# ChristianFeldmann/libHM

Hardware: AMD Instinct MI355X
Metric: decoded Mpixels/s (luma), 2160p Main10 reconstruction + loop filters (higher is better)
Workload: dtype int16 samples / int32 accumulate; 1 GPU; 3840x2160 Main10 lowdelay_P pictures, pre-parsed CTU metadata: prep+MC+dequant/IT/recon+deblock+SAO, batch of 16 independent pictures per step, inputs resident in HBM; sub_benchmark=full, streams=2, parallelism=frame-parallel, 1 process per GPU, no data-path collective

## Files before the change

libhm_amd/csrc/filter_core.h:

```cpp
#pragma once
#include "hmgpu_dev.h"

namespace hmgpu {

static __constant__ uint8_t c_tc_table[54] = {0, 0, 0, 0, 0, 0, 0, 0, 0, 0, 0, 0, 0, 0, 0, 0, 0, 0, 1, 1, 1, 1, 1, 1, 1, 1, 1,
                                       2, 2, 2, 2, 3, 3, 3, 3, 4, 4, 4, 5, 5, 6, 6, 7, 8, 9, 10, 11, 13, 14, 16, 18, 20, 22, 24};
static __constant__ uint8_t c_beta_table[52] = {0, 0, 0, 0, 0, 0, 0, 0, 0, 0, 0, 0, 0, 0, 0, 0, 6, 7, 8, 9, 10, 11, 12, 13, 14, 15,
                                         16, 17, 18, 20, 22, 24, 26, 28, 30, 32, 34, 36, 38, 40, 42, 44, 46, 48, 50, 52, 54,
                                         56, 58, 60, 62, 64};
static __constant__ uint8_t c_chroma_scale_420_dbk[58] = {
    0, 1, 2, 3, 4, 5, 6, 7, 8, 9, 10, 11, 12, 13, 14, 15, 16, 17, 18, 19, 20, 21, 22, 23, 24, 25, 26, 27, 28, 29,
    29, 30, 31, 32, 33, 33, 34, 34, 35, 35, 36, 36, 37, 37, 38, 39, 40, 41, 42, 43, 44, 45, 46, 47, 48, 49, 50, 51};

__device__ inline bool mvd4(const int16_t* a, const int16_t* b) { return abs(a[0] - b[0]) >= 4 || abs(a[1] - b[1]) >= 4; }
typedef short mv2 __attribute__((ext_vector_type(2)));
__device__ inline bool mvd4(uint32_t a, uint32_t b) {
  const mv2 d = __builtin_elementwise_sub_sat(__builtin_bit_cast(mv2, a), __builtin_bit_cast(mv2, b));
  const mv2 m = __builtin_elementwise_max(d, __builtin_elementwise_sub_sat((mv2){0, 0}, d));
  return (__builtin_bit_cast(uint32_t, m) & 0xfffcfffcu) != 0u;
}

__device__ inline int boundary_strength(const BlkInfo& p, const BlkInfo& q, bool transform_edge) {
  if ((p.flags | q.flags) & BF_INTRA) return 2;
  if (transform_edge && ((p.flags | q.flags) & BF_CBFY)) return 1;
  const int p0 = p.ref[0], p1 = p.ref[1], q0 = q.ref[0], q1 = q.ref[1];
  if ((p0 == q0 && p1 == q1) || (p0 == q1 && p1 == q0)) {
    const uint32_t pm0 = __builtin_bit_cast(uint32_t, *reinterpret_cast<const mv2*>(p.mv[0])), pm1 = __builtin_bit_cast(uint32_t, *reinterpret_cast<const mv2*>(p.mv[1]));
    const uint32_t qm0 = __builtin_bit_cast(uint32_t, *reinterpret_cast<const mv2*>(q.mv[0])), qm1 = __builtin_bit_cast(uint32_t, *reinterpret_cast<const mv2*>(q.mv[1]));
    const bool straight = mvd4(qm0, pm0) || mvd4(qm1, pm1), crossed = mvd4(qm1, pm0) || mvd4(qm0, pm1);
    if (p0 != p1) return (p0 == q0 ? straight : crossed) ? 1 : 0;
    return (straight && crossed) ? 1 : 0;
  }
  return 1;
}

typedef short s16x2 __attribute__((ext_vector_type(2)));
typedef unsigned short u16x2 __attribute__((ext_vector_type(2)));
__device__ inline s16x2 as_s16x2(uint32_t v) { return __builtin_bit_cast(s16x2, v); }
__device__ inline u16x2 as_u16x2(uint32_t v) { return __builtin_bit_cast(u16x2, v); }
__device__ inline uint32_t as_u32(s16x2 v) { return __builtin_bit_cast(uint32_t, v); }
__device__ inline uint32_t as_u32(u16x2 v) { return __builtin_bit_cast(uint32_t, v); }
__device__ inline s16x2 splat(int v) { return (s16x2){(short)v, (short)v}; }
__device__ inline u16x2 usplat(int v) { return (u16x2){(unsigned short)v, (unsigned short)v}; }
__device__ inline s16x2 pk_clip(s16x2 lo, s16x2 hi, s16x2 v) { return __builtin_elementwise_min(__builtin_elementwise_max(v, lo), hi); }

__device__ inline void filter_luma_pair_strong(uint32_t (&s)[8], int tc) {
  const u16x2 m0 = as_u16x2(s[0]), m1 = as_u16x2(s[1]), m2 = as_u16x2(s[2]), m3 = as_u16x2(s[3]);
  const u16x2 m4 = as_u16x2(s[4]), m5 = as_u16x2(s[5]), m6 = as_u16x2(s[6]), m7 = as_u16x2(s[7]);
  const s16x2 t2 = splat(2 * tc);
  const u16x2 s23 = m2 + m3, s34 = m3 + m4, s45 = m4 + m5;
  const u16x2 n3 = (m1 + s23 + s23 + m4 + m4 + m5 + usplat(4)) >> 3;
  const u16x2 n4 = (m2 + s34 + s34 + m5 + m5 + m6 + usplat(4)) >> 3;
  const u16x2 n2 = (m1 + s23 + m4 + usplat(2)) >> 2;
  const u16x2 n5 = (s34 + m5 + m6 + usplat(2)) >> 2;
  const u16x2 n1 = (m0 + m0 + m1 + m1 + m1 + s23 + m4 + usplat(4)) >> 3;
  const u16x2 n6 = (s34 + m5 + m6 + m6 + m6 + m7 + m7 + usplat(4)) >> 3;
  (void)s45;
  auto lim = [&](u16x2 m, u16x2 n) { const s16x2 c = as_s16x2(as_u32(m)); return as_u32(pk_clip(c - t2, c + t2, as_s16x2(as_u32(n)))); };
  s[1] = lim(m1, n1); s[2] = lim(m2, n2); s[3] = lim(m3, n3);
  s[4] = lim(m4, n4); s[5] = lim(m5, n5); s[6] = lim(m6, n6);
}
__device__ inline void filter_luma_pair_weak(uint32_t (&s)[8], int tc, int thr_cut, bool filt_p, bool filt_q, int maxv, bool wide) {
  const s16x2 m1 = as_s16x2(s[1]), m2 = as_s16x2(s[2]), m3 = as_s16x2(s[3]), m4 = as_s16x2(s[4]), m5 = as_s16x2(s[5]), m6 = as_s16x2(s[6]);
  const s16x2 zero = splat(0), mx = splat(maxv), tcv = splat(tc), tc2 = splat(tc >> 1);
  s16x2 delta;
  if (wide) {
    const int lo = (9 * ((int)m4.x - (int)m3.x) - 3 * ((int)m5.x - (int)m2.x) + 8) >> 4;
    const int hi = (9 * ((int)m4.y - (int)m3.y) - 3 * ((int)m5.y - (int)m2.y) + 8) >> 4;
    delta = (s16x2){(short)lo, (short)hi};
  } else {
    delta = ((m4 - m3) * splat(9) - (m5 - m2) * splat(3) + splat(8)) >> 4;
  }
  const uint32_t on = as_u32((__builtin_elementwise_max(delta, -delta) - splat(thr_cut)) >> 15);
  delta = pk_clip(-tcv, tcv, delta);
  const uint32_t n3 = as_u32(pk_clip(zero, mx, m3 + delta)), n4 = as_u32(pk_clip(zero, mx, m4 - delta));
  s[3] = (n3 & on) | (s[3] & ~on);
  s[4] = (n4 & on) | (s[4] & ~on);
  if (filt_p) {
    const s16x2 d1 = pk_clip(-tc2, tc2, ((((m1 + m3 + splat(1)) >> 1) - m2 + delta) >> 1));
    s[2] = (as_u32(pk_clip(zero, mx, m2 + d1)) & on) | (s[2] & ~on);
  }
  if (filt_q) {
    const s16x2 d2 = pk_clip(-tc2, tc2, ((((m6 + m4 + splat(1)) >> 1) - m5 - delta) >> 1));
    s[5] = (as_u32(pk_clip(zero, mx, m5 + d2)) & on) | (s[5] & ~on);
  }
}

__device__ inline void filter_luma_unit(uint32_t (&a)[8], uint32_t (&b)[8], int bs, int qp, int tc_offset_div2, int beta_offset_div2, int bd,
                                        bool p_nofilt = false, bool q_nofilt = false) {
  const int scale = 1 << (bd - 8);
  const int tc = c_tc_table[clip3(0, 53, qp + 2 * (bs - 1) + (tc_offset_div2 << 1))] * scale;
  const int beta = c_beta_table[clip3(0, 51, qp + (beta_offset_div2 << 1))] * scale;
  const int side = (beta + (beta >> 1)) >> 3;
  int l0[8], l3[8];
#pragma unroll
  for (int k = 0; k < 8; k++) { l0[k] = (int)(a[k] & 0xffffu); l3[k] = (int)(b[k] >> 16); }
  const int dp0 = abs(l0[1] - 2 * l0[2] + l0[3]), dq0 = abs(l0[4] - 2 * l0[5] + l0[6]);
  const int dp3 = abs(l3[1] - 2 * l3[2] + l3[3]), dq3 = abs(l3[4] - 2 * l3[5] + l3[6]);
  const int d0 = dp0 + dq0, d3 = dp3 + dq3, d = d0 + d3;
  if (d >= beta) return;
  const bool fp = (dp0 + dp3) < side, fq = (dq0 + dq3) < side;
  const bool s0 = (abs(l0[0] - l0[3]) + abs(l0[7] - l0[4]) < (beta >> 3)) && (2 * d0 < (beta >> 2)) &&
                  (abs(l0[3] - l0[4]) < ((tc * 5 + 1) >> 1));
  const bool s3 = (abs(l3[0] - l3[3]) + abs(l3[7] - l3[4]) < (beta >> 3)) && (2 * d3 < (beta >> 2)) &&
                  (abs(l3[3] - l3[4]) < ((tc * 5 + 1) >> 1));
  const int maxv = (1 << bd) - 1;
  uint32_t ka[8], kb[8];
#pragma unroll
  for (int k = 0; k < 8; k++) { ka[k] = a[k]; kb[k] = b[k]; }
  if (s0 && s3) {
    filter_luma_pair_strong(a, tc);
    filter_luma_pair_strong(b, tc);
  } else {
    filter_luma_pair_weak(a, tc, tc * 10, fp, fq, maxv, bd > 10);
    filter_luma_pair_weak(b, tc, tc * 10, fp, fq, maxv, bd > 10);
  }
#pragma unroll
  for (int k = 0; k < 4; k++) {
    if (p_nofilt) { a[k] = ka[k]; b[k] = kb[k]; }
    if (q_nofilt) { a[4 + k] = ka[4 + k]; b[4 + k] = kb[4 + k]; }
  }
}

__device__ inline void rows_to_pairs(const uint32_t (&r0)[4], const uint32_t (&r1)[4], uint32_t (&a)[8]) {
#pragma unroll
  for (int j = 0; j < 4; j++) {
    a[2 * j] = __builtin_amdgcn_perm(r1[j], r0[j], 0x05040100u);
    a[2 * j + 1] = __builtin_amdgcn_perm(r1[j], r0[j], 0x07060302u);
  }
}
__device__ inline void pairs_to_rows(const uint32_t (&a)[8], uint32_t (&r0)[4], uint32_t (&r1)[4]) {
#pragma unroll
  for (int j = 0; j < 4; j++) {
    r0[j] = __builtin_amdgcn_perm(a[2 * j + 1], a[2 * j], 0x05040100u);
    r1[j] = __builtin_amdgcn_perm(a[2 * j + 1], a[2 * j], 0x07060302u);
  }
}

__device__ inline int chroma_tc(int qp_avg, int pps_off, int tc_offset_div2, int bd, int fmt = 1) {
  int qp = qp_avg + pps_off;
  if (qp >= 58) qp = fmt == 1 ? qp - 6 : min(qp, 51);
  else if (qp >= 0) qp = fmt == 1 ? c_chroma_scale_420_dbk[qp] : min(qp, 51);
  return c_tc_table[clip3(0, 53, qp + 2 + (tc_offset_div2 << 1))] * (1 << (bd - 8));
}



template <int DX>
__device__ inline void shifted(const u32x4 e, uint32_t l, uint32_t r, uint32_t (&n)[4]) {
  if constexpr (DX == 0) { n[0] = e.x; n[1] = e.y; n[2] = e.z; n[3] = e.w; }
  else if constexpr (DX < 0) {
    n[0] = (e.x << 16) | l; n[1] = __builtin_amdgcn_alignbit(e.y, e.x, 16);
    n[2] = __builtin_amdgcn_alignbit(e.z, e.y, 16); n[3] = __builtin_amdgcn_alignbit(e.w, e.z, 16);
  } else {
    n[0] = __builtin_amdgcn_alignbit(e.y, e.x, 16); n[1] = __builtin_amdgcn_alignbit(e.z, e.y, 16);
    n[2] = __builtin_amdgcn_alignbit(e.w, e.z, 16); n[3] = (e.w >> 16) | (r << 16);
  }
}

__device__ inline s16x2 lut_offsets(uint32_t idx_pk, uint32_t tab_lo, uint32_t tab_hi) {
  const uint32_t looked = __builtin_amdgcn_perm(tab_hi, tab_lo, idx_pk << 8);
  return as_s16x2(__builtin_amdgcn_perm(0u, looked, 0x09030801u));
}

__device__ inline void sao_exempt_mask(const PicDev& P, int comp, int x, int row, uint32_t (&m)[4]) {
  const int sx = comp ? P.csx : 0, sy = comp ? P.csy : 0;
  const BlkInfo* g = P.blk + (size_t)((row << sy) >> 2) * P.grid_w + ((x << sx) >> 2);
#pragma unroll
  for (int j = 0; j < 4; j++) {
    const int blk = sx ? j : (j >> 1);
    m[j] = (ldg(&g[blk].flags) & BF_NOFILT) ? 0xffffffffu : 0u;
  }
}

__device__ inline u32x4 ldc8(const int16_t* row_c, int x, int comp) {
  const int16_t* p = row_c - (comp - 1) + kCStep * x;
  const u32x4 a = ldg4(p), b = ldg4(p + 8);
  const uint32_t sel = comp == 2 ? 0x07060302u : 0x05040100u;
  return u32x4{__builtin_amdgcn_perm(a.y, a.x, sel), __builtin_amdgcn_perm(a.w, a.z, sel), __builtin_amdgcn_perm(b.y, b.x, sel), __builtin_amdgcn_perm(b.w, b.z, sel)};
}
__device__ inline void stc8(int16_t* row_c, int x, const u32x4 v) {
  int16_t* p = row_c + kCStep * x;
  const uint32_t w[4] = {v.x, v.y, v.z, v.w};
#pragma unroll
  for (int j = 0; j < 4; j++) { stg(p + kCStep * 2 * j, (int16_t)(w[j] & 0xffffu)); stg(p + kCStep * (2 * j + 1), (int16_t)(w[j] >> 16)); }
}

template <int DX, int DY>
__device__ inline void sao_eo_core(int x, int row, const u32x4 cur, const uint32_t (&na)[4], const uint32_t (&nb)[4], uint32_t off_lo, uint32_t off_hi,
                                   unsigned av, int x0, int y0, int x1, int y1, int maxv, uint32_t (&out)[4]) {
  const int ya = row + DY, yb = row - DY;
  const int va = ya < y0 ? 0 : (ya > y1 ? 2 : 1), vb = yb < y0 ? 0 : (yb > y1 ? 2 : 1);
  const unsigned ra = av >> (3 * va), rb = av >> (3 * vb);
  const bool mid_ok = ((ra & rb) >> 1) & 1;
  const int last = min(7, x1 - x);
  const int ha0 = (x + DX) < x0 ? 0 : 1, hb0 = (x - DX) < x0 ? 0 : 1;
  const int hal = (x + last + DX) > x1 ? 2 : 1, hbl = (x + last - DX) > x1 ? 2 : 1;
  const bool ok0 = ((ra >> ha0) & (rb >> hb0)) & 1;
  const bool okl = ((ra >> hal) & (rb >> hbl)) & 1;
  const uint32_t c[4] = {cur.x, cur.y, cur.z, cur.w};
  const uint32_t midm = mid_ok ? 0xffffffffu : 0u;
  const uint32_t lastm = (midm & 0x0000ffffu) | (okl ? 0xffff0000u : 0u);
  uint32_t m[4] = {midm, midm, midm, midm};
  if constexpr (DX != 0) {
    m[0] = (midm & 0xffff0000u) | (ok0 ? 0x0000ffffu : 0u);
    m[1] = last == 3 ? lastm : midm;
    m[3] = last == 3 ? midm : lastm;
  }
  uint32_t one_u = 0x00010001u, mone_u = 0xffffffffu;
  asm("" : "+v"(one_u));
  asm("" : "+v"(mone_u));
  const s16x2 one = as_s16x2(one_u), mone = as_s16x2(mone_u);
#pragma unroll
  for (int j = 0; j < 4; j++) {
    const s16x2 cc = as_s16x2(c[j]);
    const s16x2 sa = __builtin_elementwise_max(__builtin_elementwise_min(cc - as_s16x2(na[j]), one), mone);
    const s16x2 sb = __builtin_elementwise_max(__builtin_elementwise_min(cc - as_s16x2(nb[j]), one), mone);
    const uint32_t et = as_u32(sa + sb + splat(2));
    const s16x2 off = lut_offsets(et, off_lo, off_hi);
    const s16x2 res = __builtin_elementwise_min(__builtin_elementwise_max(cc + off, splat(0)), splat(maxv));
    out[j] = (as_u32(res) & m[j]) | (c[j] & ~m[j]);
  }
}

}
```

libhm_amd/csrc/k_filter.hip:

```cpp
#include "hmgpu_dev.h"
#include "filter_core.h"
#include <type_traits>

namespace hmgpu {

namespace {
constexpr int kTW = 64, kTH = 64;
constexpr int kYC = kTW + 16, kYH = kTH + 8;
constexpr int kCC = kTW / 2 + 16, kCH = kTH / 2 + 4;
constexpr int kYW = kYC + 8, kCW = kCC + 8;

constexpr int kUnits = 9 * 18;
struct FilterLds {
  __attribute__((aligned(16))) int16_t y[kYH][kYW];
  __attribute__((aligned(16))) int16_t c[2][kCH][kCW];
  uint32_t unit[2][3][64];
  int32_t units[2][4];
};

struct SaoPrm { uint32_t w0, off_lo, off_hi; };
__device__ inline SaoPrm sao_fetch(const PicDev& P, int comp, int x, int row) {
  const int log2ctb = P.log2ctu - (comp ? 1 : 0);
  const int w = P.width >> (comp ? 1 : 0), h = P.height >> (comp ? 1 : 0);
  SaoPrm r = {0xffu, 0u, 0u};
  if (x < w && row < h) {
    const uint32_t* pw = reinterpret_cast<const uint32_t*>(P.saoprm + ((size_t)(row >> log2ctb) * P.ctus_w + (x >> log2ctb)) * 3 + comp);
    r.w0 = ldg(pw); r.off_lo = ldg(pw + 1); r.off_hi = ldg(pw + 2);
  }
  return r;
}

template <int W, bool NF>
__device__ inline u32x4 sao_group(const PicDev& P, int comp, const int16_t (*t)[W], int ox, int oy, int x, int row, const SaoPrm& prm) {
  const int cs = comp ? 1 : 0;
  const int w = P.width >> cs, h = P.height >> cs;
  const int log2ctb = P.log2ctu - cs;
  const int cx = x >> log2ctb, cy = row >> log2ctb;
  const uint32_t w0 = prm.w0;
  const int type = (int)(int8_t)(w0 & 0xff);
  const int16_t* line = &t[row - oy][x - ox];
  const u32x4 cur = *reinterpret_cast<const u32x4*>(line);
  if (type < 0) return cur;
  const uint32_t off_lo = prm.off_lo, off_hi = prm.off_hi;
  const int bd = P.bd[comp], maxv = (1 << bd) - 1;
  uint32_t out[4];
  if (type == HMGPU_SAO_BO) {
    const int shift = bd - 5, band0 = (w0 >> 8) & 0xff;
    const uint32_t c[4] = {cur.x, cur.y, cur.z, cur.w};
#pragma unroll
    for (int j = 0; j < 4; j++) {
      const uint32_t lo = c[j] & 0xffffu, hi = c[j] >> 16;
      const uint32_t k0 = min(((lo >> shift) - band0) & 31u, 4u), k1 = min(((hi >> shift) - band0) & 31u, 4u);
      const s16x2 off = lut_offsets(k0 | (k1 << 16), off_lo, 0u);
      out[j] = as_u32(__builtin_elementwise_min(__builtin_elementwise_max(as_s16x2(c[j]) + off, splat(0)), splat(maxv)));
    }
  } else {
    const int ctb = 1 << log2ctb;
    const int x0 = cx << log2ctb, y0 = cy << log2ctb;
    const int x1 = min(x0 + ctb, w) - 1, y1 = min(y0 + ctb, h) - 1;
    const unsigned av = w0 >> 16;
    auto run = [&](auto dxc, auto dyc) {
      constexpr int DX = decltype(dxc)::value, DY = decltype(dyc)::value;
      const int16_t* ra = line + DY * W;
      const int16_t* rb = line - DY * W;
      const u32x4 ea = *reinterpret_cast<const u32x4*>(ra), eb = *reinterpret_cast<const u32x4*>(rb);
      uint32_t na[4], nb[4];
      uint32_t la = 0, raa = 0, lb = 0, rbb = 0;
      if constexpr (DX < 0) { la = (uint16_t)ra[-1]; rbb = (uint16_t)rb[8]; }
      if constexpr (DX > 0) { raa = (uint16_t)ra[8]; lb = (uint16_t)rb[-1]; }
      shifted<DX>(ea, la, raa, na);
      shifted<-DX>(eb, lb, rbb, nb);
      sao_eo_core<DX, DY>(x, row, cur, na, nb, off_lo, off_hi, av, x0, y0, x1, y1, maxv, out);
    };
    switch (type) {
      case HMGPU_SAO_EO_0:   run(std::integral_constant<int, -1>{}, std::integral_constant<int, 0>{}); break;
      case HMGPU_SAO_EO_90:  run(std::integral_constant<int, 0>{}, std::integral_constant<int, -1>{}); break;
      case HMGPU_SAO_EO_135: run(std::integral_constant<int, -1>{}, std::integral_constant<int, -1>{}); break;
      default:               run(std::integral_constant<int, 1>{}, std::integral_constant<int, -1>{}); break;
    }
  }
  if (NF && P.any_nofilt) {
    uint32_t m[4];
    sao_exempt_mask(P, comp, x, row, m);
    const uint32_t c[4] = {cur.x, cur.y, cur.z, cur.w};
#pragma unroll
    for (int j = 0; j < 4; j++) out[j] = (c[j] & m[j]) | (out[j] & ~m[j]);
  }
  return u32x4{out[0], out[1], out[2], out[3]};
}

template <int DIR>
__device__ inline uint32_t edge_fetch(const PicDev& P, int x, int y, bool mine) {
  if (!(mine && x >= 0 && y >= 0 && x < P.width && y < P.height)) return 0u;
  const uint16_t* rec = reinterpret_cast<const uint16_t*>(P.edges + (size_t)(y >> 3) * (P.grid_w >> 1) + (x >> 3));
  return ldg(rec + (DIR == 0 ? ((y >> 2) & 1) : 2 + ((x >> 2) & 1)));
}

struct SliceLf { int tc_off, beta_off, cb_off, cr_off; };
__device__ inline SliceLf slice_lf(const SliceDev* s) {
  return {ldg(&s->tc_offset_div2), ldg(&s->beta_offset_div2), ldg(&s->pps_cb_qp_offset), ldg(&s->pps_cr_qp_offset)};
}
static_assert(HMGPU_MAX_SLICES <= 4096, "slice index must fit the 12 bits of a list entry");

template <bool NF>
__device__ inline uint32_t edge_classify(const PicDev& P, uint32_t rec, int u, int x, int y) {
  if ((rec & 3u) == 0u) return 0u;
  const uint32_t bs = rec & 3u, qp = (rec >> 2) & 127u;
  const uint32_t p_nf = NF ? (rec >> 9) & 1u : 0u, q_nf = NF ? (rec >> 10) & 1u : 0u;
  const uint32_t slice = P.slice_idx ? (uint32_t)ldg(P.slice_idx + (size_t)(y >> P.log2ctu) * P.ctus_w + (x >> P.log2ctu)) : 0u;
  return (uint32_t)u | (bs << 8) | (p_nf << 10) | (q_nf << 11) | ((qp + 32u) << 12) | (slice << 20);
}

__device__ inline void push_units(uint32_t (&list)[3][64], int32_t (&count)[4], uint32_t rec, int t) {
  const unsigned long long m = __ballot(rec != 0u);
  const int wave = t >> 6, lane = t & 63;
  if (rec != 0u) list[wave][__popcll(m & ((1ull << lane) - 1ull))] = rec;
  if (lane == 0) count[wave] = __popcll(m);
}
__device__ inline uint32_t pop_unit(const uint32_t (&list)[3][64], const int32_t (&count)[4], int t) {
  const int c0 = count[0], c1 = count[1], c2 = count[2];
  if (t < c0) return list[0][t];
  if (t < c0 + c1) return list[1][t - c0];
  if (t < c0 + c1 + c2) return list[2][t - c0 - c1];
  return 0u;
}

template <int DIR, bool NF>
__device__ inline void edge_apply(const PicDev& P, FilterLds& L, int x0, int y0, uint32_t rec, const SliceLf& s0) {
  if (rec == 0u) return;
  const int u = rec & 0xff, bs = (rec >> 8) & 3, qp = (int)((rec >> 12) & 0xff) - 64, slice = rec >> 20;
  const bool p_nf = NF && ((rec >> 10) & 1), q_nf = NF && ((rec >> 11) & 1);
  const int x = DIR == 0 ? x0 + 8 * (u % 9) : x0 - 4 + 4 * (u % 18);
  const int y = DIR == 0 ? y0 - 4 + 4 * (u / 9) : y0 + 8 * (u / 18);
  const SliceLf sl = slice == 0 ? s0 : slice_lf(P.slices + slice);
  const int tc_off = sl.tc_off, beta_off = sl.beta_off;
  int16_t* base = &L.y[y - (y0 - 4)][x - (x0 - 8)];
  uint32_t a[8], b[8];
  if (DIR == 0) {
    uint32_t r[4][4];
#pragma unroll
    for (int i = 0; i < 4; i++) {
      const u32x2 lo = *reinterpret_cast<const u32x2*>(base + i * kYW - 4), hi = *reinterpret_cast<const u32x2*>(base + i * kYW);
      r[i][0] = lo.x; r[i][1] = lo.y; r[i][2] = hi.x; r[i][3] = hi.y;
    }
    rows_to_pairs(r[0], r[1], a);
    rows_to_pairs(r[2], r[3], b);
  } else {
#pragma unroll
    for (int k = 0; k < 8; k++) {
      const u32x2 v = *reinterpret_cast<const u32x2*>(base + (k - 4) * kYW);
      a[k] = v.x; b[k] = v.y;
    }
  }
  filter_luma_unit(a, b, bs, qp, tc_off, beta_off, P.bd[0], p_nf, q_nf);
  if (DIR == 0) {
    uint32_t r[4][4];
    pairs_to_rows(a, r[0], r[1]);
    pairs_to_rows(b, r[2], r[3]);
#pragma unroll
    for (int i = 0; i < 4; i++) {
      *reinterpret_cast<u32x2*>(base + i * kYW - 4) = (u32x2){r[i][0], r[i][1]};
      *reinterpret_cast<u32x2*>(base + i * kYW) = (u32x2){r[i][2], r[i][3]};
    }
  } else {
#pragma unroll
    for (int k = 1; k < 7; k++) *reinterpret_cast<u32x2*>(base + (k - 4) * kYW) = (u32x2){a[k], b[k]};
  }
  if (bs == 2 && ((DIR == 0 ? x : y) & 15) == 0 && !P.mono) {
    const int maxc = (1 << P.bd[1]) - 1;
#pragma unroll
    for (int comp = 1; comp < 3; comp++) {
      const int tc = chroma_tc(qp, comp == 1 ? sl.cb_off : sl.cr_off, tc_off, P.bd[comp]);
      int16_t* cb = &L.c[comp - 1][(y >> 1) - ((y0 >> 1) - 2)][(x >> 1) - ((x0 >> 1) - 8)];
#pragma unroll
      for (int i = 0; i < 2; i++) {
        int16_t* s = DIR == 0 ? cb + i * kCW : cb + i;
        const int o = DIR == 0 ? 1 : kCW;
        const int m2 = (uint16_t)s[-2 * o], m3 = (uint16_t)s[-o], m4 = (uint16_t)s[0], m5 = (uint16_t)s[o];
        const int delta = clip3(-tc, tc, ((((m4 - m3) << 2) + m2 - m5 + 4) >> 3));
        if (!p_nf) s[-o] = (int16_t)clip3(0, maxc, m3 + delta);
        if (!q_nf) s[0] = (int16_t)clip3(0, maxc, m4 - delta);
      }
    }
  }
}

}

template <bool NF>
__global__ void __launch_bounds__(256) k_filter_fused(const PicDev* __restrict__ pics, Batch b, int tiles_x, int tiles) {
  __shared__ FilterLds L;
  int slot, lb;
  if (!xcd_remap(blockIdx.x, b.n, tiles, slot, lb)) return;
  const PicDev& P = pics[b.pic[slot]];
  const int x0 = (lb % tiles_x) * kTW, y0 = (lb / tiles_x) * kTH;
  const int t = threadIdx.x;
  const int vx = x0 + 8 * (t % 9), vy = y0 - 4 + 4 * (t / 9), hx = x0 - 4 + 4 * (t % 18), hy = y0 + 8 * (t / 18);
  const uint32_t ev = edge_fetch<0>(P, vx, vy, t < kUnits), eh = edge_fetch<1>(P, hx, hy, t < kUnits);
  const SliceLf s0 = slice_lf(P.slices);
  int lx[2], ly[2];
  SaoPrm sl[2];
#pragma unroll
  for (int k = 0; k < 2; k++) {
    const int g = t + 256 * k;
    lx[k] = x0 + (g & 7) * 8; ly[k] = y0 + (g >> 3);
    sl[k] = sao_fetch(P, 0, lx[k], ly[k]);
  }
  const int ccomp = 1 + (t & 1), ccx = (x0 >> 1) + ((t >> 1) & 3) * 8, ccy = (y0 >> 1) + (t >> 3);
  const SaoPrm sc = sao_fetch(P, ccomp, ccx, ccy);
  constexpr int VPR = kYC / 8, VPC = kCC / 8, NY = (kYH * VPR + 255) / 256, NC = (2 * kCH * VPC + 255) / 256;
  u32x4 ty[NY], tc[NC];
  {
    const int16_t* src = P.rec[0] + (ptrdiff_t)(y0 - 4) * P.pitch[0] + (x0 - 8);
#pragma unroll
    for (int k = 0; k < NY; k++) {
      const int i = t + 256 * k, r = i / VPR, v = i % VPR;
      if (i < kYH * VPR) ty[k] = ldg4(src + (ptrdiff_t)r * P.pitch[0] + 8 * v);
    }
#pragma unroll
    for (int k = 0; k < NC; k++) {
      const int i = t + 256 * k, r = i / (2 * VPC), v = i % (2 * VPC);
      if (i < 2 * kCH * VPC) tc[k] = ldg4(P.rec[1] + (ptrdiff_t)((y0 >> 1) - 2 + r) * P.pitch[1] + kCStep * (((x0 >> 1) - 8) + 4 * v));
    }
  }
  if (t < 192) {
    push_units(L.unit[0], L.units[0], edge_classify<NF>(P, ev, t, vx, vy), t);
    push_units(L.unit[1], L.units[1], edge_classify<NF>(P, eh, t, hx, hy), t);
  }
#pragma unroll
  for (int k = 0; k < NY; k++) {
    const int i = t + 256 * k, r = i / VPR, v = i % VPR;
    if (i < kYH * VPR) *reinterpret_cast<u32x4*>(&L.y[r][8 * v]) = ty[k];
  }
#pragma unroll
  for (int k = 0; k < NC; k++) {
    const int i = t + 256 * k, r = i / (2 * VPC), v = i % (2 * VPC);
    if (i < 2 * kCH * VPC) {
      *reinterpret_cast<u32x2*>(&L.c[0][r][4 * v]) = u32x2{__builtin_amdgcn_perm(tc[k].y, tc[k].x, 0x05040100u), __builtin_amdgcn_perm(tc[k].w, tc[k].z, 0x05040100u)};
      *reinterpret_cast<u32x2*>(&L.c[1][r][4 * v]) = u32x2{__builtin_amdgcn_perm(tc[k].y, tc[k].x, 0x07060302u), __builtin_amdgcn_perm(tc[k].w, tc[k].z, 0x07060302u)};
    }
  }
  __syncthreads();
  edge_apply<0, NF>(P, L, x0, y0, pop_unit(L.unit[0], L.units[0], t), s0);
  __syncthreads();
  edge_apply<1, NF>(P, L, x0, y0, pop_unit(L.unit[1], L.units[1], t), s0);
  __syncthreads();
#pragma unroll
  for (int k = 0; k < 2; k++)
    if (lx[k] < P.width && ly[k] < P.height)
      stg4(P.sao[0] + (size_t)ly[k] * P.pitch[0] + lx[k], sao_group<kYW, NF>(P, 0, L.y, x0 - 8, y0 - 4, lx[k], ly[k], sl[k]));
  if (ccx < (P.width >> 1) && ccy < (P.height >> 1)) {
    const u32x4 own = sao_group<kCW, NF>(P, ccomp, L.c[ccomp - 1], (x0 >> 1) - 8, (y0 >> 1) - 2, ccx, ccy, sc);
    const bool odd = t & 1;
    const uint32_t r0 = (uint32_t)__shfl_xor((int)(odd ? own.x : own.z), 1, 64), r1 = (uint32_t)__shfl_xor((int)(odd ? own.y : own.w), 1, 64);
    const uint32_t cb0 = odd ? r0 : own.x, cb1 = odd ? r1 : own.y, cr0 = odd ? own.z : r0, cr1 = odd ? own.w : r1;
    const u32x4 o = {__builtin_amdgcn_perm(cr0, cb0, 0x05040100u), __builtin_amdgcn_perm(cr0, cb0, 0x07060302u),
                     __builtin_amdgcn_perm(cr1, cb1, 0x05040100u), __builtin_amdgcn_perm(cr1, cb1, 0x07060302u)};
    stg4(P.sao[1] + (size_t)ccy * P.pitch[1] + kCStep * (ccx + (odd ? 4 : 0)), o);
  }
}

void launch_filter_fused(const PicDev* pics, const Batch& b, int width, int height, bool nofilt, hipStream_t s) {
  const int tiles_x = (width + kTW - 1) / kTW, tiles = tiles_x * ((height + kTH - 1) / kTH);
  dim3 grid((unsigned)xcd_grid(b.n, tiles));
  if (nofilt) hipLaunchKernelGGL(k_filter_fused<true>, grid, dim3(256), 0, s, pics, b, tiles_x, tiles);
  else hipLaunchKernelGGL(k_filter_fused<false>, grid, dim3(256), 0, s, pics, b, tiles_x, tiles);
}

}
```

Baseline: 180,400 Mpixels/s.

## Use buffer loads/stores and scalar-cached picture state in fused filter kernel

```diff
diff --git a/libhm_amd/csrc/filter_core.h b/libhm_amd/csrc/filter_core.h
--- a/libhm_amd/csrc/filter_core.h
+++ b/libhm_amd/csrc/filter_core.h
@@ -163,7 +163,8 @@
   return as_s16x2(__builtin_amdgcn_perm(0u, looked, 0x09030801u));
 }
 
-__device__ inline void sao_exempt_mask(const PicDev& P, int comp, int x, int row, uint32_t (&m)[4]) {
+template <typename PIC>
+__device__ inline void sao_exempt_mask(const PIC& P, int comp, int x, int row, uint32_t (&m)[4]) {
   const int sx = comp ? P.csx : 0, sy = comp ? P.csy : 0;
   const BlkInfo* g = P.blk + (size_t)((row << sy) >> 2) * P.grid_w + ((x << sx) >> 2);
 #pragma unroll
diff --git a/libhm_amd/csrc/k_filter.hip b/libhm_amd/csrc/k_filter.hip
--- a/libhm_amd/csrc/k_filter.hip
+++ b/libhm_amd/csrc/k_filter.hip
@@ -18,20 +18,56 @@
   int32_t units[2][4];
 };
 
+struct SliceLf { int tc_off, beta_off, cb_off, cr_off; };
+struct FPic {
+  static constexpr int csx = 1, csy = 1;
+  int width, height, bd0, bd1, bd2, log2ctu, ctus_w, pitch[2], grid_w, any_nofilt, mono;
+  __device__ inline int bd(int comp) const { return comp == 0 ? bd0 : comp == 1 ? bd1 : bd2; }
+  const int16_t* rec[2];
+  int16_t* sao[2];
+  const uint16_t* slice_idx;
+  const SliceDev* slices;
+  const BlkInfo* blk;
+  const EdgeRec* edges;
+  const SaoDev* saoprm;
+  SliceLf s0;
+};
+template <typename T> __device__ inline T ldc(const T* p) { return *(const T __attribute__((address_space(4)))*)p; }
+__device__ inline FPic pic_state(const PicDev* p) {
+  FPic f;
+  f.width = ldc(&p->width); f.height = ldc(&p->height);
+  f.bd0 = ldc(&p->bd[0]); f.bd1 = ldc(&p->bd[1]); f.bd2 = ldc(&p->bd[2]);
+  f.log2ctu = ldc(&p->log2ctu); f.ctus_w = ldc(&p->ctus_w);
+  f.pitch[0] = ldc(&p->pitch[0]); f.pitch[1] = ldc(&p->pitch[1]);
+  f.grid_w = ldc(&p->grid_w);
+  f.rec[0] = ldc(&p->rec[0]); f.rec[1] = ldc(&p->rec[1]);
+  f.sao[0] = ldc(&p->sao[0]); f.sao[1] = ldc(&p->sao[1]);
+  f.any_nofilt = ldc(&p->any_nofilt); f.mono = ldc(&p->mono);
+  f.slice_idx = ldc(&p->slice_idx); f.slices = ldc(&p->slices);
+  f.blk = ldc(&p->blk); f.edges = ldc(&p->edges); f.saoprm = ldc(&p->saoprm);
+  const SliceDev* s = f.slices;
+  f.s0 = {ldc(&s->tc_offset_div2), ldc(&s->beta_offset_div2), ldc(&s->pps_cb_qp_offset), ldc(&s->pps_cr_qp_offset)};
+  return f;
+}
+
+struct Span {
+  __amdgpu_buffer_rsrc_t rs;
+  uint32_t bytes;
+  __device__ inline Span(const void* base, uint32_t n) : rs(__builtin_amdgcn_make_buffer_rsrc(const_cast<void*>(base), 0, n, 0x00020000)), bytes(n) {}
+  __device__ inline uint32_t at(bool valid, uint32_t off) const { return valid ? off : bytes; }
+  __device__ inline u32x4 load4(uint32_t off) const { return __builtin_bit_cast(u32x4, __builtin_amdgcn_raw_buffer_load_b128(rs, off, 0, 0)); }
+  __device__ inline uint32_t load_u16(uint32_t off) const { return (uint16_t)__builtin_amdgcn_raw_buffer_load_b16(rs, off, 0, 0); }
+  __device__ inline void store4(uint32_t off, u32x4 v) const { __builtin_amdgcn_raw_buffer_store_b128(__builtin_bit_cast(decltype(__builtin_amdgcn_raw_buffer_load_b128(rs, 0, 0, 0)), v), rs, off, 0, 0); }
+};
+
 struct SaoPrm { uint32_t w0, off_lo, off_hi; };
-__device__ inline SaoPrm sao_fetch(const PicDev& P, int comp, int x, int row) {
-  const int log2ctb = P.log2ctu - (comp ? 1 : 0);
-  const int w = P.width >> (comp ? 1 : 0), h = P.height >> (comp ? 1 : 0);
-  SaoPrm r = {0xffu, 0u, 0u};
-  if (x < w && row < h) {
-    const uint32_t* pw = reinterpret_cast<const uint32_t*>(P.saoprm + ((size_t)(row >> log2ctb) * P.ctus_w + (x >> log2ctb)) * 3 + comp);
-    r.w0 = ldg(pw); r.off_lo = ldg(pw + 1); r.off_hi = ldg(pw + 2);
-  }
-  return r;
+__device__ inline SaoPrm sao_fetch(const Span& sp, uint32_t off) {
+  const auto v = __builtin_amdgcn_raw_buffer_load_b96(sp.rs, off, 0, 0);
+  return {(uint32_t)v[0], (uint32_t)v[1], (uint32_t)v[2]};
 }
 
 template <int W, bool NF>
-__device__ inline u32x4 sao_group(const PicDev& P, int comp, const int16_t (*t)[W], int ox, int oy, int x, int row, const SaoPrm& prm) {
+__device__ inline u32x4 sao_group(const FPic& P, int comp, const int16_t (*t)[W], int ox, int oy, int x, int row, const SaoPrm& prm) {
   const int cs = comp ? 1 : 0;
   const int w = P.width >> cs, h = P.height >> cs;
   const int log2ctb = P.log2ctu - cs;
@@ -42,7 +78,7 @@
   const u32x4 cur = *reinterpret_cast<const u32x4*>(line);
   if (type < 0) return cur;
   const uint32_t off_lo = prm.off_lo, off_hi = prm.off_hi;
-  const int bd = P.bd[comp], maxv = (1 << bd) - 1;
+  const int bd = P.bd(comp), maxv = (1 << bd) - 1;
   uint32_t out[4];
   if (type == HMGPU_SAO_BO) {
     const int shift = bd - 5, band0 = (w0 >> 8) & 0xff;
@@ -89,26 +125,17 @@
   return u32x4{out[0], out[1], out[2], out[3]};
 }
 
-template <int DIR>
-__device__ inline uint32_t edge_fetch(const PicDev& P, int x, int y, bool mine) {
-  if (!(mine && x >= 0 && y >= 0 && x < P.width && y < P.height)) return 0u;
-  const uint16_t* rec = reinterpret_cast<const uint16_t*>(P.edges + (size_t)(y >> 3) * (P.grid_w >> 1) + (x >> 3));
-  return ldg(rec + (DIR == 0 ? ((y >> 2) & 1) : 2 + ((x >> 2) & 1)));
-}
-
-struct SliceLf { int tc_off, beta_off, cb_off, cr_off; };
 __device__ inline SliceLf slice_lf(const SliceDev* s) {
   return {ldg(&s->tc_offset_div2), ldg(&s->beta_offset_div2), ldg(&s->pps_cb_qp_offset), ldg(&s->pps_cr_qp_offset)};
 }
 static_assert(HMGPU_MAX_SLICES <= 4096, "slice index must fit the 12 bits of a list entry");
 
 template <bool NF>
-__device__ inline uint32_t edge_classify(const PicDev& P, uint32_t rec, int u, int x, int y) {
-  if ((rec & 3u) == 0u) return 0u;
+__device__ inline uint32_t edge_classify(uint32_t rec, uint32_t slice, int u) {
   const uint32_t bs = rec & 3u, qp = (rec >> 2) & 127u;
   const uint32_t p_nf = NF ? (rec >> 9) & 1u : 0u, q_nf = NF ? (rec >> 10) & 1u : 0u;
-  const uint32_t slice = P.slice_idx ? (uint32_t)ldg(P.slice_idx + (size_t)(y >> P.log2ctu) * P.ctus_w + (x >> P.log2ctu)) : 0u;
-  return (uint32_t)u | (bs << 8) | (p_nf << 10) | (q_nf << 11) | ((qp + 32u) << 12) | (slice << 20);
+  const uint32_t e = (uint32_t)u | (bs << 8) | (p_nf << 10) | (q_nf << 11) | ((qp + 32u) << 12) | (slice << 20);
+  return bs ? e : 0u;
 }
 
 __device__ inline void push_units(uint32_t (&list)[3][64], int32_t (&count)[4], uint32_t rec, int t) {
@@ -126,13 +153,13 @@
 }
 
 template <int DIR, bool NF>
-__device__ inline void edge_apply(const PicDev& P, FilterLds& L, int x0, int y0, uint32_t rec, const SliceLf& s0) {
+__device__ inline void edge_apply(const FPic& P, FilterLds& L, int x0, int y0, uint32_t rec) {
   if (rec == 0u) return;
   const int u = rec & 0xff, bs = (rec >> 8) & 3, qp = (int)((rec >> 12) & 0xff) - 64, slice = rec >> 20;
   const bool p_nf = NF && ((rec >> 10) & 1), q_nf = NF && ((rec >> 11) & 1);
   const int x = DIR == 0 ? x0 + 8 * (u % 9) : x0 - 4 + 4 * (u % 18);
   const int y = DIR == 0 ? y0 - 4 + 4 * (u / 9) : y0 + 8 * (u / 18);
-  const SliceLf sl = slice == 0 ? s0 : slice_lf(P.slices + slice);
+  const SliceLf sl = slice == 0 ? P.s0 : slice_lf(P.slices + slice);
   const int tc_off = sl.tc_off, beta_off = sl.beta_off;
   int16_t* base = &L.y[y - (y0 - 4)][x - (x0 - 8)];
   uint32_t a[8], b[8];
@@ -152,7 +179,7 @@
       a[k] = v.x; b[k] = v.y;
     }
   }
-  filter_luma_unit(a, b, bs, qp, tc_off, beta_off, P.bd[0], p_nf, q_nf);
+  filter_luma_unit(a, b, bs, qp, tc_off, beta_off, P.bd(0), p_nf, q_nf);
   if (DIR == 0) {
     uint32_t r[4][4];
     pairs_to_rows(a, r[0], r[1]);
@@ -167,10 +194,10 @@
     for (int k = 1; k < 7; k++) *reinterpret_cast<u32x2*>(base + (k - 4) * kYW) = (u32x2){a[k], b[k]};
   }
   if (bs == 2 && ((DIR == 0 ? x : y) & 15) == 0 && !P.mono) {
-    const int maxc = (1 << P.bd[1]) - 1;
+    const int maxc = (1 << P.bd(1)) - 1;
 #pragma unroll
     for (int comp = 1; comp < 3; comp++) {
-      const int tc = chroma_tc(qp, comp == 1 ? sl.cb_off : sl.cr_off, tc_off, P.bd[comp]);
+      const int tc = chroma_tc(qp, comp == 1 ? sl.cb_off : sl.cr_off, tc_off, P.bd(comp));
       int16_t* cb = &L.c[comp - 1][(y >> 1) - ((y0 >> 1) - 2)][(x >> 1) - ((x0 >> 1) - 8)];
 #pragma unroll
       for (int i = 0; i < 2; i++) {
@@ -192,71 +219,75 @@
   __shared__ FilterLds L;
   int slot, lb;
   if (!xcd_remap(blockIdx.x, b.n, tiles, slot, lb)) return;
-  const PicDev& P = pics[b.pic[slot]];
+  const FPic P = pic_state(pics + b.pic[slot]);
+  __builtin_amdgcn_sched_barrier(0);
   const int x0 = (lb % tiles_x) * kTW, y0 = (lb / tiles_x) * kTH;
   const int t = threadIdx.x;
+  const int l2 = P.log2ctu, p0 = P.pitch[0], p1 = P.pitch[1];
   const int vx = x0 + 8 * (t % 9), vy = y0 - 4 + 4 * (t / 9), hx = x0 - 4 + 4 * (t % 18), hy = y0 + 8 * (t / 18);
-  const uint32_t ev = edge_fetch<0>(P, vx, vy, t < kUnits), eh = edge_fetch<1>(P, hx, hy, t < kUnits);
-  const SliceLf s0 = slice_lf(P.slices);
-  int lx[2], ly[2];
-  SaoPrm sl[2];
-#pragma unroll
-  for (int k = 0; k < 2; k++) {
-    const int g = t + 256 * k;
-    lx[k] = x0 + (g & 7) * 8; ly[k] = y0 + (g >> 3);
-    sl[k] = sao_fetch(P, 0, lx[k], ly[k]);
-  }
-  const int ccomp = 1 + (t & 1), ccx = (x0 >> 1) + ((t >> 1) & 3) * 8, ccy = (y0 >> 1) + (t >> 3);
-  const SaoPrm sc = sao_fetch(P, ccomp, ccx, ccy);
-  constexpr int VPR = kYC / 8, VPC = kCC / 8, NY = (kYH * VPR + 255) / 256, NC = (2 * kCH * VPC + 255) / 256;
-  u32x4 ty[NY], tc[NC];
-  {
-    const int16_t* src = P.rec[0] + (ptrdiff_t)(y0 - 4) * P.pitch[0] + (x0 - 8);
-#pragma unroll
-    for (int k = 0; k < NY; k++) {
-      const int i = t + 256 * k, r = i / VPR, v = i % VPR;
-      if (i < kYH * VPR) ty[k] = ldg4(src + (ptrdiff_t)r * P.pitch[0] + 8 * v);
-    }
-#pragma unroll
-    for (int k = 0; k < NC; k++) {
-      const int i = t + 256 * k, r = i / (2 * VPC), v = i % (2 * VPC);
-      if (i < 2 * kCH * VPC) tc[k] = ldg4(P.rec[1] + (ptrdiff_t)((y0 >> 1) - 2 + r) * P.pitch[1] + kCStep * (((x0 >> 1) - 8) + 4 * v));
-    }
-  }
+  const bool vin = t < kUnits && vy >= 0 && vx < P.width && vy < P.height, hin = t < kUnits && hx >= 0 && hx < P.width && hy < P.height;
+  const int ecw = P.grid_w >> 1, ex0 = (x0 >> 3) - 1, ey0 = (y0 >> 3) - 1;
+  const Span se(reinterpret_cast<const char*>(P.edges) + ((ptrdiff_t)ey0 * ecw + ex0) * (ptrdiff_t)sizeof(EdgeRec), (uint32_t)((9 * ecw + 10) * (int)sizeof(EdgeRec)));
+  const uint32_t ev = se.load_u16(se.at(vin, (uint32_t)((((vy >> 3) - ey0) * ecw + (vx >> 3) - ex0) * 8 + ((vy >> 2) & 1) * 2)));
+  const uint32_t eh = se.load_u16(se.at(hin, (uint32_t)((((hy >> 3) - ey0) * ecw + (hx >> 3) - ex0) * 8 + 4 + ((hx >> 2) & 1) * 2)));
+  const int sx0 = (x0 - 8) >> l2, sy0 = (y0 - 8) >> l2;
+  const Span ss(reinterpret_cast<const char*>(P.slice_idx) + ((ptrdiff_t)sy0 * P.ctus_w + sx0) * 2,
+                P.slice_idx ? (uint32_t)(((((y0 + 64) >> l2) - sy0) * P.ctus_w + ((x0 + 64) >> l2) - sx0 + 1) * 2) : 0u);
+  uint32_t sv = ss.load_u16(ss.at(vin, (uint32_t)((((vy >> l2) - sy0) * P.ctus_w + (vx >> l2) - sx0) * 2)));
+  uint32_t sh = ss.load_u16(ss.at(hin, (uint32_t)((((hy >> l2) - sy0) * P.ctus_w + (hx >> l2) - sx0) * 2)));
+  constexpr int VPR = kYC / 8, VPC = 2 * kCC / 8;
+  static_assert(kYH * VPR > 512 && kYH * VPR <= 768 && kCH * VPC > 256 && kCH * VPC <= 512, "three rounds of luma vectors, two of chroma");
+  const int yr0 = t / VPR, yv0 = t % VPR, yr1 = (t + 256) / VPR, yv1 = (t + 256) % VPR, yr2 = (t + 512) / VPR, yv2 = (t + 512) % VPR;
+  const int ur0 = t / VPC, uv0 = t % VPC, ur1 = (t + 256) / VPC, uv1 = (t + 256) % VPC;
+  const bool yin2 = t + 512 < kYH * VPR, uin1 = t + 256 < kCH * VPC;
+  const Span sy(P.rec[0] + ((ptrdiff_t)(y0 - 4) * p0 + (x0 - 8)), (uint32_t)(((kYH - 1) * p0 + kYC) * 2));
+  const Span sc(P.rec[1] + ((ptrdiff_t)((y0 >> 1) - 2) * p1 + kCStep * ((x0 >> 1) - 8)), (uint32_t)(((kCH - 1) * p1 + kCStep * kCC) * 2));
+  const u32x4 ty0 = sy.load4((uint32_t)((yr0 * p0 + 8 * yv0) * 2));
+  const u32x4 ty1 = sy.load4((uint32_t)((yr1 * p0 + 8 * yv1) * 2));
+  const u32x4 ty2 = sy.load4(sy.at(yin2, (uint32_t)((yr2 * p0 + 8 * yv2) * 2)));
+  const u32x4 tc0 = sc.load4((uint32_t)((ur0 * p1 + 8 * uv0) * 2));
+  const u32x4 tc1 = sc.load4(sc.at(uin1, (uint32_t)((ur1 * p1 + 8 * uv1) * 2)));
+  const int gx = (t & 7) * 8, gy = t >> 3;
+  const int lx = x0 + gx, ly[2] = {y0 + gy, y0 + gy + 32};
+  const int ccomp = 1 + (t & 1), ccx = (x0 >> 1) + ((t >> 1) & 3) * 8, ccy = (y0 >> 1) + gy;
+  const bool lin[2] = {lx < P.width && ly[0] < P.height, lx < P.width && ly[1] < P.height}, cin = ccx < (P.width >> 1) && ccy < (P.height >> 1);
+  const int n64 = 63 >> l2;
+  const Span sp(P.saoprm + ((ptrdiff_t)(y0 >> l2) * P.ctus_w + (x0 >> l2)) * 3, (uint32_t)(((n64 * P.ctus_w + n64) * 3 + 3) * (int)sizeof(SaoDev)));
+  const uint32_t prow = (uint32_t)(3 * (int)sizeof(SaoDev)) * (uint32_t)P.ctus_w;
+  const SaoPrm sl0 = sao_fetch(sp, sp.at(lin[0], (uint32_t)(gy >> l2) * prow + (uint32_t)((gx >> l2) * 3 * (int)sizeof(SaoDev))));
+  const SaoPrm sl1 = sao_fetch(sp, sp.at(lin[1], (uint32_t)((gy + 32) >> l2) * prow + (uint32_t)((gx >> l2) * 3 * (int)sizeof(SaoDev))));
+  const SaoPrm sc0 = sao_fetch(sp, sp.at(cin, (uint32_t)((2 * gy) >> l2) * prow + (uint32_t)(((((t >> 1) & 3) * 16) >> l2) * 3 + ccomp) * (uint32_t)sizeof(SaoDev)));
+  asm volatile("" : "+v"(sv), "+v"(sh));
   if (t < 192) {
-    push_units(L.unit[0], L.units[0], edge_classify<NF>(P, ev, t, vx, vy), t);
-    push_units(L.unit[1], L.units[1], edge_classify<NF>(P, eh, t, hx, hy), t);
-  }
-#pragma unroll
-  for (int k = 0; k < NY; k++) {
-    const int i = t + 256 * k, r = i / VPR, v = i % VPR;
-    if (i < kYH * VPR) *reinterpret_cast<u32x4*>(&L.y[r][8 * v]) = ty[k];
-  }
-#pragma unroll
-  for (int k = 0; k < NC; k++) {
-    const int i = t + 256 * k, r = i / (2 * VPC), v = i % (2 * VPC);
-    if (i < 2 * kCH * VPC) {
-      *reinterpret_cast<u32x2*>(&L.c[0][r][4 * v]) = u32x2{__builtin_amdgcn_perm(tc[k].y, tc[k].x, 0x05040100u), __builtin_amdgcn_perm(tc[k].w, tc[k].z, 0x05040100u)};
-      *reinterpret_cast<u32x2*>(&L.c[1][r][4 * v]) = u32x2{__builtin_amdgcn_perm(tc[k].y, tc[k].x, 0x07060302u), __builtin_amdgcn_perm(tc[k].w, tc[k].z, 0x07060302u)};
-    }
-  }
+    push_units(L.unit[0], L.units[0], edge_classify<NF>(ev, sv, t), t);
+    push_units(L.unit[1], L.units[1], edge_classify<NF>(eh, sh, t), t);
+  }
+  *reinterpret_cast<u32x4*>(&L.y[yr0][8 * yv0]) = ty0;
+  *reinterpret_cast<u32x4*>(&L.y[yr1][8 * yv1]) = ty1;
+  if (yin2) *reinterpret_cast<u32x4*>(&L.y[yr2][8 * yv2]) = ty2;
+  auto put_chroma = [&](int r, int v, const u32x4 c) {
+    *reinterpret_cast<u32x2*>(&L.c[0][r][4 * v]) = u32x2{__builtin_amdgcn_perm(c.y, c.x, 0x05040100u), __builtin_amdgcn_perm(c.w, c.z, 0x05040100u)};
+    *reinterpret_cast<u32x2*>(&L.c[1][r][4 * v]) = u32x2{__builtin_amdgcn_perm(c.y, c.x, 0x07060302u), __builtin_amdgcn_perm(c.w, c.z, 0x07060302u)};
+  };
+  put_chroma(ur0, uv0, tc0);
+  if (uin1) put_chroma(ur1, uv1, tc1);
   __syncthreads();
-  edge_apply<0, NF>(P, L, x0, y0, pop_unit(L.unit[0], L.units[0], t), s0);
+  edge_apply<0, NF>(P, L, x0, y0, pop_unit(L.unit[0], L.units[0], t));
   __syncthreads();
-  edge_apply<1, NF>(P, L, x0, y0, pop_unit(L.unit[1], L.units[1], t), s0);
+  edge_apply<1, NF>(P, L, x0, y0, pop_unit(L.unit[1], L.units[1], t));
   __syncthreads();
-#pragma unroll
-  for (int k = 0; k < 2; k++)
-    if (lx[k] < P.width && ly[k] < P.height)
-      stg4(P.sao[0] + (size_t)ly[k] * P.pitch[0] + lx[k], sao_group<kYW, NF>(P, 0, L.y, x0 - 8, y0 - 4, lx[k], ly[k], sl[k]));
-  if (ccx < (P.width >> 1) && ccy < (P.height >> 1)) {
-    const u32x4 own = sao_group<kCW, NF>(P, ccomp, L.c[ccomp - 1], (x0 >> 1) - 8, (y0 >> 1) - 2, ccx, ccy, sc);
+  const Span oy(P.sao[0] + ((ptrdiff_t)y0 * p0 + x0), (uint32_t)(((kTH - 1) * p0 + kTW) * 2));
+  if (lin[0]) oy.store4((uint32_t)((gy * p0 + gx) * 2), sao_group<kYW, NF>(P, 0, L.y, x0 - 8, y0 - 4, lx, ly[0], sl0));
+  if (lin[1]) oy.store4((uint32_t)(((gy + 32) * p0 + gx) * 2), sao_group<kYW, NF>(P, 0, L.y, x0 - 8, y0 - 4, lx, ly[1], sl1));
+  if (cin) {
+    const u32x4 own = sao_group<kCW, NF>(P, ccomp, L.c[ccomp - 1], (x0 >> 1) - 8, (y0 >> 1) - 2, ccx, ccy, sc0);
     const bool odd = t & 1;
     const uint32_t r0 = (uint32_t)__shfl_xor((int)(odd ? own.x : own.z), 1, 64), r1 = (uint32_t)__shfl_xor((int)(odd ? own.y : own.w), 1, 64);
     const uint32_t cb0 = odd ? r0 : own.x, cb1 = odd ? r1 : own.y, cr0 = odd ? own.z : r0, cr1 = odd ? own.w : r1;
     const u32x4 o = {__builtin_amdgcn_perm(cr0, cb0, 0x05040100u), __builtin_amdgcn_perm(cr0, cb0, 0x07060302u),
                      __builtin_amdgcn_perm(cr1, cb1, 0x05040100u), __builtin_amdgcn_perm(cr1, cb1, 0x07060302u)};
-    stg4(P.sao[1] + (size_t)ccy * P.pitch[1] + kCStep * (ccx + (odd ? 4 : 0)), o);
+    const Span oc(P.sao[1] + ((ptrdiff_t)(y0 >> 1) * p1 + kCStep * (x0 >> 1)), (uint32_t)(((kTH / 2 - 1) * p1 + kCStep * kTW / 2) * 2));
+    oc.store4((uint32_t)((gy * p1 + kCStep * (((t >> 1) & 3) * 8 + (odd ? 4 : 0))) * 2), o);
   }
 }
 
```

New measurement: 190,300 Mpixels/s (median of 6 runs). 1.05x the previous value.
